# ecpoppenheimer/TensorFlowRayTrace

Hardware: AMD Instinct MI355X
Metric: ray-surface intersection tests/sec (fwd+bwd) (higher is better)
Workload: dtype f32 ray state, f32 filter + f64 decisions

## Files before the change

### tensorflowraytrace_amd/csrc/tfrt_trace3d.hip

```cpp
#include <vector>

#include <type_traits>
#include "tfrt_common.h"
#include "goal_finish.h"
#include "wave_schedule.h"

namespace tfrt {

constexpr int TILE = 512;
constexpr int KC = 24;

constexpr int ERR_CAPACITY = 1;


__global__ __launch_bounds__(BLOCK) void k_center(const double* __restrict__ fverts, int M,
                                                  double* __restrict__ c0, int32_t* nrays0, int n,
                                                  int32_t* tail8, unsigned int* scan_ticket) {
  if (nrays0 != nullptr) {
    if (threadIdx.x == 0) *nrays0 = n;
    if (threadIdx.x < 8) tail8[threadIdx.x] = 0;
    if (threadIdx.x == 0 && scan_ticket != nullptr) *scan_ticket = 0u;
  }
  __shared__ double red[WAVES][3];
  __shared__ double ctr[3];
// ... 1102 lines not shown
  group_walk<T, 1, false>(rays, stride, *n_ptr, last_tri, susphere, clsphere, csphere, crec, cface,
                          fverts, c0, prep, pstride, n_clusters, chunk_clusters, eps_int, eps_size,
                          eps_start, part_t, part_i, part_stride, catagory, rec_tri, rec_t, rec_cls,
                          blockcnt, nullptr, (int)blockIdx.x * BLOCK, -1);
}

template <typename T>
__global__ __launch_bounds__(BLOCK) void k_intersect_group_left(
    const T* __restrict__ rays, int64_t stride, const int32_t* __restrict__ n_ptr,
    const int32_t* __restrict__ last_tri, const float4* __restrict__ susphere,
    const float4* __restrict__ clsphere, const float4* __restrict__ csphere,
    const float4* __restrict__ crec, const int32_t* __restrict__ cface,
    const double* __restrict__ fverts, const double* __restrict__ c0, int n_clusters,
    int chunk_clusters, double eps_int, double eps_size, double eps_start,
    const int32_t* __restrict__ catagory, int32_t* __restrict__ rec_tri,
    double* __restrict__ rec_t, uint8_t* __restrict__ rec_cls,
    const int32_t* __restrict__ left_list, const int32_t* __restrict__ left_count,
    int32_t* __restrict__ hist) {
  const int n = *n_ptr;
  const int total = *left_count;
  for (int item = blockIdx.x; item * WAVES < total; item += gridDim.x) {
    const int k = item * WAVES + (int)(threadIdx.x >> 6);
    const int qwave = k < total ? left_list[k] : -1;
    group_walk<T, 1, true>(rays, stride, n, last_tri, susphere, clsphere, csphere, crec, cface,
                           fverts, c0, nullptr, 0, n_clusters, chunk_clusters, eps_int, eps_size,
                           eps_start, nullptr, nullptr, 0, catagory, rec_tri, rec_t, rec_cls,
                           nullptr, hist, 0, qwave);
    __syncthreads();
  }
}

constexpr int BEAM_SLIST = 64;
constexpr int BEAM_CLIST = 32;
constexpr int BEAM_FLIST = 192;
constexpr int BEAM_WIDE = 48;

struct Beam {
  float ox, oy, oz, wx, wy, wz, R0, S, tmin;
  float e1x, e1y, e1z, e2x, e2y, e2z;
  float R0b, tb;
  __device__ __forceinline__ float radius(float t, float pad) const {
    return fminf(R0 + S * (fabsf(t) + pad), R0b + S * (fabsf(t - tb) + pad));
  }
};

__device__ __forceinline__ bool beam_touch(const Beam& b, const float4 sp) {
  const float r = __builtin_amdgcn_sqrtf(sp.w) * 1.000002f;
  const float vx = sp.x - b.ox, vy = sp.y - b.oy, vz = sp.z - b.oz;
  const float t = vx * b.wx + vy * b.wy + vz * b.wz;
  const float v2 = vx * vx + vy * vy + vz * vz;
  const float B = r + b.radius(t, r);
  return (v2 - t * t <= B * B + 2e-6f * v2) && !(t + r < b.tmin);
}

__device__ __forceinline__ bool face_frame(const Beam& b, const float4 r0, const float4 r1,
                                           const float4 r2, const float es, float4 rec[4]) {
  const float n1 = fabsf(r1.x) + fabsf(r1.y) + fabsf(r1.z);
  const float n2 = fabsf(r2.x) + fabsf(r2.y) + fabsf(r2.z);
  const float scale = fabsf(r0.x) + fabsf(r0.y) + fabsf(r0.z) + fabsf(b.ox) + fabsf(b.oy) +
                      fabsf(b.oz) + n1 + n2;
  const float slack = 5.05f * es * (n1 + n2) + 8e-6f * scale;
  const float ax = r0.x - b.ox, ay = r0.y - b.oy, az = r0.z - b.oz;
  const float t0 = ax * b.wx + ay * b.wy + az * b.wz;
  const float t1 = t0 + (r1.x * b.wx + r1.y * b.wy + r1.z * b.wz);
  const float t2 = t0 + (r2.x * b.wx + r2.y * b.wy + r2.z * b.wz);
  const float tlo = fminf(t0, fminf(t1, t2)) - slack, thi = fmaxf(t0, fmaxf(t1, t2)) + slack;
  const float q0x = ax * b.e1x + ay * b.e1y + az * b.e1z, q0y = ax * b.e2x + ay * b.e2y + az * b.e2z;
  const float g1x = r1.x * b.e1x + r1.y * b.e1y + r1.z * b.e1z,
              g1y = r1.x * b.e2x + r1.y * b.e2y + r1.z * b.e2z;
  const float g2x = r2.x * b.e1x + r2.y * b.e1y + r2.z * b.e1z,
              g2y = r2.x * b.e2x + r2.y * b.e2y + r2.z * b.e2z;
  const float area = g1x * g2y - g1y * g2x;
  const float l1 = g1x * g1x + g1y * g1y, l2 = g2x * g2x + g2y * g2y;
  const bool flat = !(area * area > 1e-8f * l1 * l2);
  const float sg = area > 0.f ? 1.f : -1.f;
  auto edge = [&](float px, float py, float dx, float dy, float* nx, float* ny, float* c) {
    const float k = sg * __builtin_amdgcn_rsqf(dx * dx + dy * dy);
    *nx = dy * k;
    *ny = -dx * k;
    *c = -(*nx * px + *ny * py);
  };
  float nx0, ny0, c0, nx1, ny1, c1, nx2, ny2, c2;
  edge(q0x, q0y, g1x, g1y, &nx0, &ny0, &c0);
  edge(q0x + g1x, q0y + g1y, g2x - g1x, g2y - g1y, &nx1, &ny1, &c1);
  edge(q0x + g2x, q0y + g2y, -g2x, -g2y, &nx2, &ny2, &c2);
  if (flat) {
    nx0 = ny0 = nx1 = ny1 = nx2 = ny2 = 0.f;
    c0 = c1 = c2 = -INFINITY;
  }
  const float slack2 = 1.5f * slack;
  rec[0] = make_float4(nx0, ny0, c0, tlo);
  rec[1] = make_float4(nx1, ny1, c1, thi);
  rec[2] = make_float4(nx2, ny2, c2, 0.5f * (tlo + thi));
  rec[3] = make_float4(0.5001f * (thi - tlo), slack2, r0.w, 0.f);
  const float rho = (fminf(b.R0 + b.S * fmaxf(fabsf(tlo), fabsf(thi)),
                           b.R0b + b.S * fmaxf(fabsf(tlo - b.tb), fabsf(thi - b.tb))) +
                     slack2) * 1.0001f;
  return !(c0 > rho) && !(c1 > rho) && !(c2 > rho) && !(thi < b.tmin);
}

template <typename Op>
__device__ __forceinline__ float wave_reduce_f(float v, Op op) {
  auto dpp = [](float x, auto ctrl, auto row_mask) {
    return __int_as_float(__builtin_amdgcn_update_dpp(__float_as_int(x), __float_as_int(x),
                                                      decltype(ctrl)::value,
                                                      decltype(row_mask)::value, 0xF, false));
  };
  using std::integral_constant;
  v = op(v, dpp(v, integral_constant<int, 0xB1>{}, integral_constant<int, 0xF>{}));
  v = op(v, dpp(v, integral_constant<int, 0x4E>{}, integral_constant<int, 0xF>{}));
  v = op(v, dpp(v, integral_constant<int, 0x141>{}, integral_constant<int, 0xF>{}));
  v = op(v, dpp(v, integral_constant<int, 0x140>{}, integral_constant<int, 0xF>{}));
  v = op(v, dpp(v, integral_constant<int, 0x142>{}, integral_constant<int, 0xA>{}));
  v = op(v, dpp(v, integral_constant<int, 0x143>{}, integral_constant<int, 0xC>{}));
  return __int_as_float(__builtin_amdgcn_readlane(__float_as_int(v), 63));
}
__device__ __forceinline__ float wave_sum_f(float v) {
  return wave_reduce_f(v, [](float a, float b) { return a + b; });
}
__device__ __forceinline__ float wave_max_f(float v) {
  return wave_reduce_f(v, [](float a, float b) { return fmaxf(a, b); });
}
__device__ __forceinline__ float wave_min_f(float v) {
  return wave_reduce_f(v, [](float a, float b) { return fminf(a, b); });
}
#define TFRT_DPP_STEP4(OPA, OPB, OPC, OPD, CTRL)      \
  OPA " %0, %0, %0 " CTRL "\n\t" OPB " %1, %1, %1 " CTRL "\n\t" \
  OPC " %2, %2, %2 " CTRL "\n\t" OPD " %3, %3, %3 " CTRL "\n\t"
#define TFRT_DPP_ALL4(OPA, OPB, OPC, OPD)                                        \
  "s_nop 1\n\t"                                                                  \
  TFRT_DPP_STEP4(OPA, OPB, OPC, OPD, "quad_perm:[1,0,3,2] row_mask:0xf bank_mask:0xf") \
  TFRT_DPP_STEP4(OPA, OPB, OPC, OPD, "quad_perm:[2,3,0,1] row_mask:0xf bank_mask:0xf") \
  TFRT_DPP_STEP4(OPA, OPB, OPC, OPD, "row_half_mirror row_mask:0xf bank_mask:0xf")     \
  TFRT_DPP_STEP4(OPA, OPB, OPC, OPD, "row_mirror row_mask:0xf bank_mask:0xf")          \
  TFRT_DPP_STEP4(OPA, OPB, OPC, OPD, "row_bcast:15 row_mask:0xa bank_mask:0xf")        \
  TFRT_DPP_STEP4(OPA, OPB, OPC, OPD, "row_bcast:31 row_mask:0xc bank_mask:0xf")
__device__ __forceinline__ void wave_sum4(float& a, float& b, float& c, float& d) {
  __asm__ volatile(TFRT_DPP_ALL4("v_add_f32_dpp", "v_add_f32_dpp", "v_add_f32_dpp", "v_add_f32_dpp")
                   : "+v"(a), "+v"(b), "+v"(c), "+v"(d));
  a = __int_as_float(__builtin_amdgcn_readlane(__float_as_int(a), 63));
  b = __int_as_float(__builtin_amdgcn_readlane(__float_as_int(b), 63));
  c = __int_as_float(__builtin_amdgcn_readlane(__float_as_int(c), 63));
  d = __int_as_float(__builtin_amdgcn_readlane(__float_as_int(d), 63));
}
__device__ __forceinline__ void wave_max3_min(float& a, float& b, float& c, float& d) {
  __asm__ volatile(TFRT_DPP_ALL4("v_max_f32_dpp", "v_max_f32_dpp", "v_max_f32_dpp", "v_min_f32_dpp")
                   : "+v"(a), "+v"(b), "+v"(c), "+v"(d));
  a = __int_as_float(__builtin_amdgcn_readlane(__float_as_int(a), 63));
  b = __int_as_float(__builtin_amdgcn_readlane(__float_as_int(b), 63));
  c = __int_as_float(__builtin_amdgcn_readlane(__float_as_int(c), 63));
  d = __int_as_float(__builtin_amdgcn_readlane(__float_as_int(d), 63));
}

__device__ __forceinline__ float uniform_f(float v) {
  return __int_as_float(__builtin_amdgcn_readfirstlane(__float_as_int(v)));
}
__device__ __forceinline__ float bcast_f(float v, int src_lane) {
  return __int_as_float(__builtin_amdgcn_readlane(__float_as_int(v), src_lane));
}

template <typename U>
using LdsPtr = __attribute__((address_space(3))) U*;

template <typename RT>
__device__ __forceinline__ void beam_decide(const int nb, const int lane, LdsPtr<const uint32_t> x_pair,
                                         LdsPtr<const RT> rt, LdsPtr<unsigned long long> best_k,
                                         LdsPtr<int32_t> best_i, const double* __restrict__ fverts,
                                         const double eps_int, const double eps_size,
                                         const double eps_start) {
  bool have = false;
  unsigned long long key = 0, old = 0;
  int j = -1;
  const uint32_t xp = lane < nb ? x_pair[lane] : 0u;
  const int slot = (int)(xp & 63u);
  if (lane < nb) {
    double s[3], e[3];
#pragma unroll
    for (int k = 0; k < 3; ++k) {
      s[k] = static_cast<double>(rt[k * 64 + slot]);
      e[k] = static_cast<double>(rt[(3 + k) * 64 + slot]);
    }
    j = (int)(xp >> 6);
    old = best_k[slot];
    double P[9];
    const double* fp = fverts + 9 * (int64_t)j;
#pragma unroll
    for (int k = 0; k < 9; ++k) P[k] = fp[k];
    const TriHit h = exact_triangle(s, e, P, eps_int, eps_size, eps_start);
    if (h.valid) {
      have = true;
      key = dkey(h.ray_u);
    }
  }
  wave_fence();
  if (have) atomicMin((unsigned long long*)&best_k[slot], key);
  wave_fence();
  bool win = false;
  if (have) {
    const unsigned long long now = best_k[slot];
    win = key == now;
    if (win && now < old) best_i[slot] = 0x7FFFFFFF;
  }
  wave_fence();
  if (win) atomicMin((int32_t*)&best_i[slot], j);
  wave_fence();
}

template <typename RT>
struct BeamLds {
  uint16_t slist[BEAM_SLIST];
  uint16_t clist[BEAM_CLIST];
  uint32_t flist[BEAM_FLIST];
  uint32_t x_pair[192];
  float4 ftab[64][4];
  RT rtab[6][64];
  unsigned long long best_k[64];
  int32_t best_i[64];
};

struct BeamScene {
  const float4* susphere;
  const float4* clsphere;
  const float4* csphere;
  const float4* crec;
  const double* fverts;
  const double* c0;
  int n_clusters, n_super;
  double eps_int, eps_size, eps_start;
};

#ifdef TFRT_TICKS
#define TFRT_WI_ARG _wi
#else
#define TFRT_WI_ARG nullptr
#endif

template <typename T, typename RT>
__device__ __forceinline__ bool beam_pass(BeamLds<RT>& W, const BeamScene& g, const int lane,
                                          const int bundle, const bool live, const int skip,
                                          const bool first_pass, const int coherent_only,
                                          unsigned* _wi, unsigned* work = nullptr) {
  TFRT_TICK_INIT;
  const float4* __restrict__ susphere = g.susphere;
  const float4* __restrict__ clsphere = g.clsphere;
  const float4* __restrict__ csphere = g.csphere;
  const float4* __restrict__ crec = g.crec;
  const double* __restrict__ fverts = g.fverts;
  const double* __restrict__ c0 = g.c0;
  const int n_clusters = g.n_clusters, n_super = g.n_super;
  const double eps_int = g.eps_int, eps_size = g.eps_size, eps_start = g.eps_start;
  const float4 never = make_float4(0.f, 0.f, 0.f, -1.f);
  W.best_k[lane] = dkey(INFINITY);
  W.best_i[lane] = -1;
  const double cx = c0[0], cy = c0[1], cz = c0[2];
  const float cxf = uniform_f((float)cx), cyf = uniform_f((float)cy), czf = uniform_f((float)cz);
  auto rel = [](const RT v, const double c, const float cf) -> float {
    if constexpr (sizeof(T) <= 4) return (float)v - cf;
    else return (float)((double)v - c);
  };
  const float es_f = (float)eps_size;
  int xn = 0;

  auto decide = [&](const int nb) {
    TFRT_STAT(28, 1);
    TFRT_WAVE_NOTE(1, 1);
    wave_fence();
    beam_decide<RT>(nb, lane, (LdsPtr<const uint32_t>)&W.x_pair[0],
                    (LdsPtr<const RT>)&W.rtab[0][0], (LdsPtr<unsigned long long>)&W.best_k[0],
                    (LdsPtr<int32_t>)&W.best_i[0], fverts, eps_int, eps_size, eps_start);
  };

  TFRT_STAT(8, 1);
  constexpr int BEAM_ATTEMPTS = 20;
  TFRT_TICK(0);
  float gap = -1.f;
  unsigned long long cuts = 0ull;
  int lo = 0, attempts = 0;
  bool spread = false;
  while (lo < bundle) {
    ++attempts;
    TFRT_STAT(30, 1);
    TFRT_WAVE_NOTE(0, 1);
    const unsigned long long above = lo < 63 ? (cuts >> (lo + 1)) << (lo + 1) : 0ull;
    const int hi = above != 0ull ? __ffsll((long long)above) - 1 : bundle;
    const int len = hi - lo;
    wave_fence();
    RT own[6];
#pragma unroll
    for (int k = 0; k < 6; ++k) own[k] = W.rtab[k][lane];
    const float sx = rel(own[0], cx, cxf), sy = rel(own[1], cy, cyf), sz = rel(own[2], cz, czf);
    const float dx = (float)(own[3] - own[0]), dy = (float)(own[4] - own[1]),
                dz = (float)(own[5] - own[2]);
    const float len2 = dx * dx + dy * dy + dz * dz;
    const bool ok = live && len2 > 0.f && len2 < 3.0e38f;
    const float inv = ok ? __builtin_amdgcn_rsqf(len2) : 0.f;
    const float ux = dx * inv, uy = dy * inv, uz = dz * inv;
    const float rabs = fabsf(sx) + fabsf(sy) + fabsf(sz);
    const bool sel = ok && lane >= lo && lane < hi;
    const float4 su_first = lane < n_super ? susphere[lane] : never;
    const float cnt = (float)__popcll(__ballot(sel));
    bool narrow = true, brute = false;
    int ns = 0, nc = 0, nf = 0;
    Beam bm = {0.f, 0.f, 0.f, 0.f, 0.f, 1.f, 0.f, 0.f, -INFINITY, 1.f, 0.f, 0.f, 0.f, 1.f, 0.f,
               INFINITY, 0.f};
    float ray_t = 0.f, ray_dt = 0.f, ray_terr = 0.f;
    float Ax = 0.f, Ay = 0.f, Mx = 0.f, My = 0.f, Mlen = 0.f, Perr = 0.f, Pm = 0.f;
    if (cnt > 0.f) {
      float swx = sel ? ux : 0.f, swy = sel ? uy : 0.f, swz = sel ? uz : 0.f;
      float sox = sel ? sx : 0.f, soy = sel ? sy : 0.f, soz = sel ? sz : 0.f;
      float pad0 = 0.f, pad1 = 0.f;
      wave_sum4(swx, swy, swz, sox);
      wave_sum4(soy, soz, pad0, pad1);
      const float wl2 = swx * swx + swy * swy + swz * swz;
      narrow = wl2 > 0.49f * cnt * cnt;
      spread = !narrow;
      const float wi = narrow ? __builtin_amdgcn_rsqf(wl2) : 0.f;
      bm.wx = swx * wi; bm.wy = swy * wi; bm.wz = swz * wi;
      const float icnt = __builtin_amdgcn_rcpf(cnt);
      bm.ox = sox * icnt; bm.oy = soy * icnt; bm.oz = soz * icnt;
      const float cosk = ux * bm.wx + uy * bm.wy + uz * bm.wz;
      if (__any(sel && !(cosk > 0.7f))) narrow = false, spread = true;
      const float px = sx - bm.ox, py = sy - bm.oy, pz = sz - bm.oz;
      const float ts = px * bm.wx + py * bm.wy + pz * bm.wz;
      ray_t = ts;
      ray_dt = dx * bm.wx + dy * bm.wy + dz * bm.wz;
      ray_terr = 1e-5f * (rabs + fabsf(bm.ox) + fabsf(bm.oy) + fabsf(bm.oz));
      {
        const float f0 = fabsf(bm.wx), f1 = fabsf(bm.wy), f2 = fabsf(bm.wz);
        const bool k0 = f0 <= f1 && f0 <= f2, k1 = !k0 && f1 <= f2;
        const float kx = k0 ? 1.f : 0.f, ky = k1 ? 1.f : 0.f, kz = (!k0 && !k1) ? 1.f : 0.f;
        const float cxx = bm.wy * kz - bm.wz * ky, cyy = bm.wz * kx - bm.wx * kz,
                    czz = bm.wx * ky - bm.wy * kx;
        const float il = __builtin_amdgcn_rsqf(cxx * cxx + cyy * cyy + czz * czz);
        bm.e1x = cxx * il; bm.e1y = cyy * il; bm.e1z = czz * il;
        bm.e2x = bm.wy * bm.e1z - bm.wz * bm.e1y;
        bm.e2y = bm.wz * bm.e1x - bm.wx * bm.e1z;
        bm.e2z = bm.wx * bm.e1y - bm.wy * bm.e1x;
      }
      {
        const float idt = __builtin_amdgcn_rcpf(sel ? ray_dt : 1.f);
        Mx = (dx * bm.e1x + dy * bm.e1y + dz * bm.e1z) * idt;
        My = (dx * bm.e2x + dy * bm.e2y + dz * bm.e2z) * idt;
        const float p1 = px * bm.e1x + py * bm.e1y + pz * bm.e1z,
                    p2 = px * bm.e2x + py * bm.e2y + pz * bm.e2z;
        Ax = p1 - ts * Mx;
        Ay = p2 - ts * My;
        Mlen = __builtin_amdgcn_sqrtf(Mx * Mx + My * My) * 1.0001f;
        Pm = 2e-5f * (fabsf(Mx) + fabsf(My));
        Perr = 2e-5f * (fabsf(p1) + fabsf(p2) + fabsf(ts) * (fabsf(Mx) + fabsf(My)) + rabs +
                        fabsf(bm.ox) + fabsf(bm.oy) + fabsf(bm.oz));
      }
      float R0 = sel ? __builtin_amdgcn_sqrtf(Ax * Ax + Ay * Ay) : 0.f, S = sel ? Mlen : 0.f;
      float Lw = sel ? rabs : 0.f, tmin = sel ? ts : INFINITY;
      wave_max3_min(R0, S, Lw, tmin);
      Lw += fabsf(bm.ox) + fabsf(bm.oy) + fabsf(bm.oz);
      const float tb = -(bm.ox * bm.wx + bm.oy * bm.wy + bm.oz * bm.wz);
      float R0b = 0.f;
      if (sel) {
        const float bx = Ax + Mx * tb, by = Ay + My * tb;
        R0b = __builtin_amdgcn_sqrtf(bx * bx + by * by);
      }
      R0b = wave_max_f(R0b);
      bm.R0 = R0 * 1.001f + 4e-6f * Lw;
      bm.S = S * 1.001f + 2e-6f;
      bm.tb = tb;
      bm.R0b = R0b * 1.001f + 4e-6f * (Lw + fabsf(tb)) + 2e-6f * fabsf(tb) * S;
      if (!(bm.R0b < 3.0e38f)) bm.R0b = INFINITY;
      bm.tmin = (!first_pass && eps_start >= 0.0) ? tmin - 1e-5f * Lw - 1e-5f * fabsf(tmin)
                                                  : -INFINITY;
      if (!(bm.R0 < 3.0e38f && bm.S < 3.0e38f)) narrow = false;
      bm.ox = uniform_f(bm.ox); bm.oy = uniform_f(bm.oy); bm.oz = uniform_f(bm.oz);
      bm.wx = uniform_f(bm.wx); bm.wy = uniform_f(bm.wy); bm.wz = uniform_f(bm.wz);
      bm.R0 = uniform_f(bm.R0); bm.S = uniform_f(bm.S); bm.tmin = uniform_f(bm.tmin);
      bm.R0b = uniform_f(bm.R0b); bm.tb = uniform_f(bm.tb);
      bm.e1x = uniform_f(bm.e1x); bm.e1y = uniform_f(bm.e1y); bm.e1z = uniform_f(bm.e1z);
      bm.e2x = uniform_f(bm.e2x); bm.e2y = uniform_f(bm.e2y); bm.e2z = uniform_f(bm.e2z);
      TFRT_TICK(1);

      if (narrow) {
        float4 nxt = su_first;
        for (int b = 0; b < n_super; b += 64) {
          const int node = b + lane;
          const float4 cur = nxt;
          nxt = node + 64 < n_super ? susphere[node + 64] : never;
          const bool hit = beam_touch(bm, cur);
          const unsigned long long m = __ballot(hit);
          if (hit) {
            const int pos = ns + rank_below(m);
            if (pos < BEAM_SLIST) W.slist[pos] = (uint16_t)node;
          }
          ns += __popcll(m);
        }
        narrow = ns <= BEAM_SLIST && n_super <= 65536;
      }
      wave_fence();
      TFRT_TICK(2);
      if (narrow && ns > 0) {
        for (int b = 0; b < ns * SUPER; b += 64) {
          const int k = b + lane;
          bool hit = false;
          int cl = 0;
          if (k < ns * SUPER) {
            cl = (int)W.slist[k >> 3] * SUPER + (k & 7);
            if (cl < n_clusters) hit = beam_touch(bm, clsphere[cl]);
          }
          const unsigned long long m = __ballot(hit);
          if (hit) {
            const int pos = nc + rank_below(m);
            if (pos < BEAM_CLIST) W.clist[pos] = (uint16_t)cl;
          }
          nc += __popcll(m);
        }
        narrow = nc <= BEAM_CLIST && n_clusters <= 65536;
      }
      wave_fence();
      TFRT_TICK(3);
      if (narrow && nc > 0) {
        for (int b = 0; b < nc * CLUSTER; b += 64) {
          const int k = b + lane;
          bool hit = false;
          unsigned slot = 0;
          if (k < nc * CLUSTER) {
            slot = (unsigned)W.clist[k >> 4] * CLUSTER + (unsigned)(k & 15);
            hit = beam_touch(bm, csphere[slot]);
          }
          const unsigned long long m = __ballot(hit);
          if (hit) {
            const int pos = nf + rank_below(m);
            if (pos < BEAM_FLIST) W.flist[pos] = slot;
          }
          nf += __popcll(m);
        }
        narrow = nf <= BEAM_FLIST && !(nf > BEAM_WIDE && len > 8 && attempts <= 6);
      }
      wave_fence();
      TFRT_TICK(4);
    }
    if (!narrow) {
      TFRT_TICK(10);
      const bool hopeless = !coherent_only &&
                            ((len == bundle && (spread || (nc > 64 && nc > n_clusters / 4))) ||
                             attempts >= BEAM_ATTEMPTS);
      if (len > 1 && !hopeless) {
        if (cuts == 0ull) {
          const float su = sx * ux + sy * uy + sz * uz;
          const float fx = sx - su * ux, fy = sy - su * uy, fz = sz - su * uz;
          const float gx = fx - __shfl_up(fx, 1, 64), gy = fy - __shfl_up(fy, 1, 64),
                      gz = fz - __shfl_up(fz, 1, 64);
          const float hx = ux - __shfl_up(ux, 1, 64), hy = uy - __shfl_up(uy, 1, 64),
                      hz = uz - __shfl_up(uz, 1, 64);
          const bool prev_ok = __shfl_up(ok ? 1 : 0, 1, 64) != 0;
          gap = 0.f;
          if (ok && prev_ok && lane > 0)
            gap = gx * gx + gy * gy + gz * gz +
                  (sx * sx + sy * sy + sz * sz) * (hx * hx + hy * hy + hz * hz);
          if (!(gap >= 0.f)) gap = 0.f;
        }
        const bool inside = lane > lo && lane < hi;
        const float widest = wave_max_f(inside ? gap : -1.f);
        const unsigned long long at = __ballot(inside && gap == widest);
        const int g = (widest > 0.f && at != 0ull) ? __ffsll((long long)at) - 1 : lo + (len >> 1);
        cuts |= 1ull << g;
        continue;
      }
      if (len == 1 && !hopeless) {
        brute = true;
      } else {
        TFRT_STAT(ns > BEAM_SLIST ? 10 : (nc > BEAM_CLIST ? 11 : (nf > BEAM_FLIST ? 12 : 9)), 1);
        TFRT_STAT(15, lo);
        return false;
      }
    }

    TFRT_STAT(13, nf);
    TFRT_WAVE_NOTE(3, nf);
    TFRT_TICK(5);
    auto reach_now = [&]() {
      const double best = dkey_inv(W.best_k[lane]);
      const float bu = nextafterf((float)best, INFINITY) * ray_dt;
      return ray_t + bu + 1e-5f * fabsf(bu) + ray_terr;
    };
    float myreach = reach_now();
    bool queued = false;
    const int n_cand = brute ? n_clusters * CLUSTER : nf;
    int f0 = 0;
    do {
      const int nb = min(64, n_cand - f0);
      if (work != nullptr) work[1] += (unsigned)nb;
      float4 rec[4] = {never, never, never, never};
      bool touch = false;
      float tnear = INFINITY;
      bool cand = lane < nb;
      if (brute && cand) {
        const float4 sp = csphere[f0 + lane];
        const float vx = sp.x - bm.ox, vy = sp.y - bm.oy, vz = sp.z - bm.oz;
        const float vu = vx * bm.wx + vy * bm.wy + vz * bm.wz;
        const float v2 = vx * vx + vy * vy + vz * vz;
        const float rr = __builtin_amdgcn_sqrtf(sp.w) * 1.000002f + bm.radius(vu, 0.f);
        cand = v2 - vu * vu <= rr * rr + 4e-6f * v2;
      }
      if (cand) {
        const int64_t memb = brute ? (int64_t)(f0 + lane) : (int64_t)W.flist[f0 + lane];
        const float4 r0 = crec[3 * memb], r1 = crec[3 * memb + 1], r2 = crec[3 * memb + 2];
        touch = face_frame(bm, r0, r1, r2, es_f, rec) && __float_as_int(r0.w) >= 0;
        tnear = rec[0].w;
        if (tnear != tnear) tnear = -INFINITY;
        rec[0].w = tnear;
      }
      f0 += 64;
      const bool closing = f0 >= n_cand && hi == bundle;
      const unsigned long long tm = __ballot(touch);
      const int nt = __popcll(tm);
      int place = 0;
      for (unsigned long long rest = tm; rest != 0ull; rest &= rest - 1ull) {
        const int o = __ffsll((long long)rest) - 1;
        const float to = bcast_f(tnear, o);
        place += (to < tnear || (to == tnear && o < lane)) ? 1 : 0;
      }
      wave_fence();
      if (touch) {
        W.ftab[place][0] = rec[0];
        W.ftab[place][1] = rec[1];
        W.ftab[place][2] = rec[2];
        W.ftab[place][3] = rec[3];
      }
      wave_fence();
      TFRT_STAT(27, nt);
      TFRT_TICK(6);
      float span = -INFINITY;
      auto on_face = [&](const float word, const int b, int* j, float* thi) {
        const float tn = bcast_f(word, b + 3), tc = bcast_f(word, b + 11);
        *thi = bcast_f(word, b + 7);
        *j = __float_as_int(bcast_f(word, b + 14));
        const float ix = Ax + Mx * tc, iy = Ay + My * tc;
        const float room = Mlen * bcast_f(word, b + 12) + bcast_f(word, b + 13) + Perr + Pm * fabsf(tc);
        return sel && *j != skip && !(myreach < tn) &&
               !(bm.tmin > -INFINITY && *thi < ray_t - ray_terr) &&
               !(bcast_f(word, b) * ix + bcast_f(word, b + 1) * iy + bcast_f(word, b + 2) > room) &&
               !(bcast_f(word, b + 4) * ix + bcast_f(word, b + 5) * iy + bcast_f(word, b + 6) > room) &&
               !(bcast_f(word, b + 8) * ix + bcast_f(word, b + 9) * iy + bcast_f(word, b + 10) > room);
      };
      for (int c = 0;; c += 2) {
        const bool end = c >= nt;
        const bool two = c + 1 < nt;
        const float word =
            reinterpret_cast<const float*>(&W.ftab[end ? 0 : c][0])[lane & (two ? 31 : 15)];
        const float tn = end ? INFINITY : bcast_f(word, 3);
        const bool flush =
            end ? closing
                : (tn > span && __ballot(sel && !(queued || myreach < INFINITY)) == 0ull);
        while (xn >= 64 || (flush && xn > 0)) {
          const int nd = min(xn, 64);
          wave_fence();
          decide(nd);
          uint32_t tp = 0u, tq = 0u;
          if (lane < xn - nd) tp = W.x_pair[nd + lane];
          if (lane + 64 < xn - nd) tq = W.x_pair[nd + 64 + lane];
          wave_fence();
          if (lane < xn - nd) W.x_pair[lane] = tp;
          if (lane + 64 < xn - nd) W.x_pair[64 + lane] = tq;
          xn -= nd;
          wave_fence();
          if (xn == 0) queued = false;
          myreach = reach_now();
          TFRT_TICK(8);
        }
        if (end) break;
        if (__ballot(sel && !(myreach < tn)) == 0ull) {
          c = nt - 2;
          continue;
        }
        TFRT_STAT(29, two ? 2 : 1);
        TFRT_WAVE_NOTE(2, two ? 2 : 1);
        int ja, jb = -1;
        float thia, thib = -INFINITY;
        const bool keepa = on_face(word, 0, &ja, &thia);
        bool keepb = false;
        if (two) keepb = on_face(word, 16, &jb, &thib);
        span = fmaxf(span, fmaxf(thia, thib));
        const unsigned long long kma = __ballot(keepa), kmb = __ballot(keepb);
        const int na = __popcll(kma);
        if (keepa) W.x_pair[xn + rank_below(kma)] = ((uint32_t)ja << 6) | (uint32_t)lane;
        if (keepb) W.x_pair[xn + na + rank_below(kmb)] = ((uint32_t)jb << 6) | (uint32_t)lane;
        queued = queued || keepa || keepb;
        xn += na + __popcll(kmb);
        if (work != nullptr) work[0] += (unsigned)(na + __popcll(kmb));
        TFRT_STAT(14, na + __popcll(kmb));
        TFRT_TICK(7);
      }
    } while (f0 < n_cand);
    lo = hi;
  }
  wave_fence();
  return true;
}

template <typename T, int BW>
__global__ __launch_bounds__(64 * BW) void k_intersect_beam(
    const T* __restrict__ rays, int64_t stride, const int32_t* __restrict__ n_ptr,
    const int32_t* __restrict__ last_tri, BeamScene g, const int32_t* __restrict__ catagory,
    int32_t* __restrict__ rec_tri, double* __restrict__ rec_t, uint8_t* __restrict__ rec_cls,
    int32_t* __restrict__ hist, int32_t* __restrict__ left_list, int32_t* __restrict__ left_count,
    int32_t* __restrict__ left_total, int coherent_only, int bundle) {
  const int tid = threadIdx.x, lane = tid & 63, wave = tid >> 6;
  const int qwave = blockIdx.x * BW + wave;
  const int q = qwave * bundle + lane;
  const int n = *n_ptr;
  if (qwave * bundle >= n) return;
  TFRT_WAVE_BEGIN;

  using RT = std::conditional_t<sizeof(T) <= 4, float, double>;
  const int i = (lane < bundle && q < n) ? q : -1;
  const bool live = i >= 0;
  const int64_t ii = live ? i : 0;
  __shared__ BeamLds<RT> lds[BW];
  BeamLds<RT>& W = lds[wave];
#pragma unroll
  for (int k = 0; k < 6; ++k) W.rtab[k][lane] = static_cast<RT>(rays[k * stride + ii]);
  const int skip = (live && last_tri != nullptr) ? last_tri[ii] : -1;
  if (!beam_pass<T, RT>(W, g, lane, bundle, live, skip, last_tri == nullptr, coherent_only,
                        TFRT_WI_ARG)) {
    if (lane == 0) {
      left_list[atomicAdd(left_count, 1)] = qwave;
      atomicAdd(left_total, 1);
    }
    return;
  }
  wave_fence();

  int cls = -1;
  if (live) {
    const int bi = W.best_i[lane];
    cls = (bi < 0) ? CLS_DEAD : cat_to_cls(catagory[bi]);
    rec_tri[i] = bi;
    rec_t[i] = dkey_inv(W.best_k[lane]);
    rec_cls[i] = (uint8_t)cls;
  }
#pragma unroll
  for (int c = 0; c < 4; ++c) {
    const int cnt_c = __popcll(__ballot(cls == c));
    if (lane == c && cnt_c > 0) atomicAdd(&hist[((qwave * bundle) >> 8) * 4 + c], cnt_c);
  }
  TFRT_WAVE_END(qwave);
}


__global__ __launch_bounds__(BLOCK) void k_classify3d(
    const int32_t* __restrict__ n_ptr, int chunks, const double* __restrict__ part_t,
    const int32_t* __restrict__ part_i, int64_t part_stride,
    const int32_t* __restrict__ catagory, int32_t* __restrict__ rec_tri,
    double* __restrict__ rec_t, uint8_t* __restrict__ rec_cls, int32_t* __restrict__ blockcnt) {
  const int n = *n_ptr;
  const int base = blockIdx.x * BLOCK;
  if (base >= n) return;
  const int i = base + threadIdx.x;
  int cls = -1;
  if (i < n) {
    double bt = INFINITY;
    int bi = -1;
    for (int c = 0; c < chunks; ++c) {
      const double t = part_t[c * part_stride + i];
      const int pi = part_i[c * part_stride + i];
      if (t < bt || (t == bt && pi >= 0 && pi < bi)) {
        bt = t;
        bi = pi;
      }
    }
    cls = (bi < 0) ? CLS_DEAD : cat_to_cls(catagory[bi]);
    rec_tri[i] = bi;
    rec_t[i] = bt;
    rec_cls[i] = (uint8_t)cls;
  }
  __shared__ int wc[WAVES][4];
  const int wave = threadIdx.x >> 6;
#pragma unroll
  for (int c = 0; c < 4; ++c) {
    const unsigned long long m = __ballot(cls == c);
    if (lane_id() == 0) wc[wave][c] = __popcll(m);
  }
  __syncthreads();
  if (threadIdx.x < 4) {
    int s = 0;
    for (int w = 0; w < WAVES; ++w) s += wc[w][threadIdx.x];
    blockcnt[blockIdx.x * 4 + threadIdx.x] = s;
  }
}


__global__ __launch_bounds__(1024) void k_scan3d_one(const int32_t* __restrict__ n_ptr,
                                                 const int32_t* __restrict__ blockcnt,
                                                 int32_t* __restrict__ blockoff,
                                                 int32_t* __restrict__ pass_counts,
                                                 int32_t* __restrict__ totals,
                                                 int32_t* __restrict__ n_next,
                                                 unsigned long long* __restrict__ n_tests,
                                                 int M) {
  const int n = *n_ptr;
  const int nblk = (n + BLOCK - 1) / BLOCK;
  __shared__ int total[4];
  scan_rows_one<4>(blockcnt, blockoff, nblk, total);
  if (threadIdx.x < 4) {
    const int c = threadIdx.x;
    pass_counts[c] = total[c];
    pass_counts[4 + c] = totals[c];
    totals[c] += total[c];
  }
  if (threadIdx.x == 0) {
    *n_next = total[CLS_ACTIVE];
    *n_tests += (unsigned long long)n * (unsigned long long)M;
  }
}

constexpr int SCAN_GRID_MIN_ROWS = 8192;
__global__ __launch_bounds__(1024) void k_scan3d(const int32_t* __restrict__ n_ptr,
                                                 const int32_t* __restrict__ blockcnt,
                                                 int32_t* __restrict__ blockoff,
                                                 int32_t* __restrict__ rowtot,
                                                 int32_t* __restrict__ rowbase,
                                                 unsigned int* __restrict__ ticket,
                                                 int32_t* __restrict__ pass_counts,
                                                 int32_t* __restrict__ totals,
                                                 int32_t* __restrict__ n_next,
                                                 unsigned long long* __restrict__ n_tests,
                                                 int M) {
  const int n = *n_ptr;
  const int nblk = (n + BLOCK - 1) / BLOCK;
  __shared__ int total[4];
  if (!scan_rows_grid<4>(blockcnt, blockoff, nblk, rowtot, rowbase, ticket, total)) return;
  if (threadIdx.x < 4) {
    const int c = threadIdx.x;
    pass_counts[c] = total[c];
// ... 2583 lines not shown
```

### tensorflowraytrace_amd/csrc/trace_math.h

```cpp
#pragma once
#include <math.h>

#if defined(__HIPCC__)
#define TFRT_HD __host__ __device__ __forceinline__
#else
#define TFRT_HD inline
#endif

namespace tfrt {

constexpr int CLS_ACTIVE = 0;
constexpr int CLS_FINISHED = 1;
constexpr int CLS_STOPPED = 2;
constexpr int CLS_DEAD = 3;

constexpr int CAT_OPTICAL = 0, CAT_STOP = 1, CAT_TARGET = 2;

struct TriHit {
  double ray_u, trig_u, trig_v;
  bool valid;
};

TFRT_HD TriHit exact_triangle(const double s[3], const double e[3], const double P[9],
                              double eps_int, double eps_size, double eps_start) {
#pragma clang fp contract(off)
  const double a = s[0] - e[0], d = s[1] - e[1], h = s[2] - e[2];
  const double b = P[3] - P[0], f = P[4] - P[1], k = P[5] - P[2];
  const double c = P[6] - P[0], g = P[7] - P[1], l = P[8] - P[2];
  const double q = s[0] - P[0], r = s[1] - P[1], t = s[2] - P[2];

  const double den = a * g * k + b * d * l + c * f * h - a * f * l - b * g * h - c * d * k;
  const double nr = b * l * r + c * f * t + g * k * q - b * g * t - c * k * r - f * l * q;
  const double nu = a * g * t + c * h * r + d * l * q - a * l * r - c * d * t - g * h * q;
  const double nv = a * k * r + b * d * t + f * h * q - a * f * t - b * h * r - d * k * q;

  TriHit o;
  bool valid = fabs(den) >= eps_int;
  const double sd = valid ? den : 1.0;
  o.ray_u = nr / sd;
  o.trig_u = nu / sd;
  o.trig_v = nv / sd;
  valid = valid && (o.trig_u >= -eps_size);
  valid = valid && (o.trig_v >= -eps_size);
  valid = valid && (o.trig_u + o.trig_v <= 1.0 + eps_size);
  valid = valid && (o.ray_u >= eps_start);
  o.valid = valid;
  return o;
}

TFRT_HD void hit_point(const double s[3], const double e[3], double ray_u, double h[3]) {
#pragma clang fp contract(off)
  h[0] = s[0] - ray_u * (s[0] - e[0]);
  h[1] = s[1] - ray_u * (s[1] - e[1]);
  h[2] = s[2] - ray_u * (s[2] - e[2]);
}

TFRT_HD double advance(double origin, double L, double dir) {
#pragma clang fp contract(off)
  return origin + L * dir;
}

TFRT_HD double advance_between(double s, double L, double e) {
#pragma clang fp contract(off)
  return s + L * (e - s);
}

TFRT_HD void cross3(const double a[3], const double b[3], double o[3]) {
#pragma clang fp contract(off)
  o[0] = a[1] * b[2] - a[2] * b[1];
  o[1] = a[2] * b[0] - a[0] * b[2];
  o[2] = a[0] * b[1] - a[1] * b[0];
}

TFRT_HD double dot3(const double a[3], const double b[3]) {
#pragma clang fp contract(off)
  return a[0] * b[0] + a[1] * b[1] + a[2] * b[2];
}

TFRT_HD void face_normal(const double P[9], double N[3], double C[3], double* clen) {
#pragma clang fp contract(off)
  const double A[3] = {P[3] - P[0], P[4] - P[1], P[5] - P[2]};
  const double B[3] = {P[6] - P[3], P[7] - P[4], P[8] - P[5]};
  cross3(A, B, C);
  const double len = sqrt(dot3(C, C));
  *clen = len;
  N[0] = C[0] / len;
  N[1] = C[1] / len;
  N[2] = C[2] / len;
}

TFRT_HD double l2_normalize3(const double v[3], double o[3]) {
#pragma clang fp contract(off)
  double sq = dot3(v, v);
  if (sq < 1e-12) sq = 1e-12;
  const double inv = 1.0 / sqrt(sq);
  o[0] = v[0] * inv;
  o[1] = v[1] * inv;
  o[2] = v[2] * inv;
  return inv;
}

struct Snell3 {
  double u[3], n[3];
  double nu, eta, k;
  bool reflect;
  double w[3];
};

TFRT_HD void snell_normal(const double P[9], double n[3]) {
  double N[3], C[3], clen;
  face_normal(P, N, C, &clen);
  l2_normalize3(N, n);
}

TFRT_HD void snell_ratios(double n_in, double n_out, double* n1, double* n2) {
#pragma clang fp contract(off)
  const bool in_safe = n_in != 0.0, out_safe = n_out != 0.0;
  const double nis = in_safe ? n_in : 1.0, nos = out_safe ? n_out : 1.0;
  *n1 = out_safe ? nis / nos : 0.0;
  *n2 = in_safe ? nos / nis : 0.0;
}

TFRT_HD Snell3 snell3d_core(const double s[3], const double h[3], const double un[3], double n1,
                            double n2, bool mirror) {
#pragma clang fp contract(off)
  Snell3 o;
  const double r[3] = {h[0] - s[0], h[1] - s[1], h[2] - s[2]};
  l2_normalize3(r, o.u);
  o.n[0] = un[0];
  o.n[1] = un[1];
  o.n[2] = un[2];
  o.nu = dot3(o.n, o.u);
  const bool internal = o.nu > 0.0;
  o.eta = internal ? n1 : n2;
  const double nu_eta = o.eta * o.nu;
  o.k = 1.0 - o.eta * o.eta + nu_eta * nu_eta;
  const bool tir = o.k < 0.0;
  o.reflect = tir || mirror;
  if (o.reflect) {
    for (int i = 0; i < 3; ++i) o.w[i] = -2.0 * o.nu * o.n[i] + o.u[i];
  } else {
    const double sg = (o.nu > 0.0) ? 1.0 : ((o.nu < 0.0) ? -1.0 : 0.0);
    const double alpha = sg * sqrt(o.k) - nu_eta;
    for (int i = 0; i < 3; ++i) o.w[i] = alpha * o.n[i] + o.eta * o.u[i];
  }
  return o;
}

TFRT_HD Snell3 snell3d_unit(const double s[3], const double h[3], const double un[3],
                            double n_in, double n_out) {
  double n1, n2;
  snell_ratios(n_in, n_out, &n1, &n2);
  return snell3d_core(s, h, un, n1, n2, n_in == 0.0);
}

TFRT_HD Snell3 snell3d(const double s[3], const double h[3], const double norm[3],
                       double n_in, double n_out) {
  double un[3];
  l2_normalize3(norm, un);
  return snell3d_unit(s, h, un, n_in, n_out);
}

TFRT_HD double fmod_floor(double x, double m) {
  double r = fmod(x, m);
  if (r != 0.0 && ((r < 0.0) != (m < 0.0))) r += m;
  return r;
}

TFRT_HD double snell2d_angle(double xs, double ys, double xe, double ye, double norm,
                             double n_in, double n_out) {
#pragma clang fp contract(off)
  const double PI = 3.141592653589793;
  norm = fmod_floor(norm, 2 * PI);
  double ray_angle = atan2(ys - ye, xs - xe);
  ray_angle = fmod_floor(ray_angle, 2 * PI);
  double theta1 = norm - ray_angle;
  if (theta1 > PI) theta1 = theta1 - 2 * PI;
  if (theta1 < -PI) theta1 = theta1 + 2 * PI;
  const bool internal = fabs(theta1) >= PI / 2;
  const bool in_safe = n_in != 0.0, out_safe = n_out != 0.0;
  const double nis = in_safe ? n_in : 1.0, nos = out_safe ? n_out : 1.0;
  const double n1 = out_safe ? nis / nos : 0.0;
  const double n2 = in_safe ? nos / nis : 0.0;
  const double n = internal ? n1 : n2;
  if (!internal) norm = norm + PI;
  if (internal) theta1 = theta1 + PI;
  const double theta2 = n * sin(theta1);
  if (fabs(theta2) <= 1.0 && n != 0.0) return norm - asin(theta2);
  return norm + theta1 + PI;
}

TFRT_HD double adj_rcp(double x) {
#if defined(__HIP_DEVICE_COMPILE__)
  double r = __builtin_amdgcn_rcp(x);
  r = __builtin_fma(__builtin_fma(-x, r, 1.0), r, r);
  r = __builtin_fma(__builtin_fma(-x, r, 1.0), r, r);
  return r;
#else
  return 1.0 / x;
#endif
// ... 179 lines not shown
```

Before: 131800 billion.

## Rewrite face culling with DPP row broadcasts and merge wave reductions

Replaces the per-face culling math, which used many readlane broadcasts, with an inline-asm sequence built on row_newbcast DPP. Each 16-lane row can then evaluate its own face record, so the second face comes from a separate 16-float load. The 64-wide ftab gets one extra padding row so that load stays in bounds. Wave reductions are regrouped so the padded sum4 and the separate R0b max collapse into a sum2+max and a single max3_min. nextafterf is replaced by a bit-trick next_up_f. The gain is fewer scalar readlanes and DPP passes in the inner candidate loop, at the cost of hand-written asm with hazard nops and stricter register-lifetime assumptions.

```diff
diff --git a/tensorflowraytrace_amd/csrc/tfrt_trace3d.hip b/tensorflowraytrace_amd/csrc/tfrt_trace3d.hip
--- a/tensorflowraytrace_amd/csrc/tfrt_trace3d.hip
+++ b/tensorflowraytrace_amd/csrc/tfrt_trace3d.hip
@@ -1278,6 +1278,53 @@
   d = __int_as_float(__builtin_amdgcn_readlane(__float_as_int(d), 63));
 }
 
+#define TFRT_DPP_STEP3(OPA, OPB, OPC, CTRL) \
+  OPA " %0, %0, %0 " CTRL "\n\t" OPB " %1, %1, %1 " CTRL "\n\t" OPC " %2, %2, %2 " CTRL "\n\t"
+#define TFRT_DPP_ALL3(OPA, OPB, OPC)                                        \
+  "s_nop 1\n\t"                                                             \
+  TFRT_DPP_STEP3(OPA, OPB, OPC, "quad_perm:[1,0,3,2] row_mask:0xf bank_mask:0xf") \
+  TFRT_DPP_STEP3(OPA, OPB, OPC, "quad_perm:[2,3,0,1] row_mask:0xf bank_mask:0xf") \
+  TFRT_DPP_STEP3(OPA, OPB, OPC, "row_half_mirror row_mask:0xf bank_mask:0xf")     \
+  TFRT_DPP_STEP3(OPA, OPB, OPC, "row_mirror row_mask:0xf bank_mask:0xf")          \
+  TFRT_DPP_STEP3(OPA, OPB, OPC, "row_bcast:15 row_mask:0xa bank_mask:0xf")        \
+  TFRT_DPP_STEP3(OPA, OPB, OPC, "row_bcast:31 row_mask:0xc bank_mask:0xf")
+__device__ __forceinline__ void wave_sum2_max(float& a, float& b, float& c) {
+  __asm__ volatile(TFRT_DPP_ALL3("v_add_f32_dpp", "v_add_f32_dpp", "v_max_f32_dpp")
+                   : "+v"(a), "+v"(b), "+v"(c));
+  a = __int_as_float(__builtin_amdgcn_readlane(__float_as_int(a), 63));
+  b = __int_as_float(__builtin_amdgcn_readlane(__float_as_int(b), 63));
+  c = __int_as_float(__builtin_amdgcn_readlane(__float_as_int(c), 63));
+}
+
+#define TFRT_BCAST(K) " row_newbcast:" #K " row_mask:0xf bank_mask:0xf\n\t"
+__device__ __forceinline__ void face_edges(const float word, const float Ax, const float Ay,
+                                           const float Mx, const float My, const float Mlen,
+                                           const float Perr, const float Pm, float& room,
+                                           float& e0, float& e1, float& e2) {
+  float ix, iy;
+  __asm__ volatile(
+      "s_nop 1\n\t"
+      "v_mov_b32_dpp %3, %6" TFRT_BCAST(11)
+      "v_mov_b32_dpp %0, %6" TFRT_BCAST(13)
+      "v_fma_f32 %5, %3, %10, %8\n\t"
+      "v_fma_f32 %4, %3, %9, %7\n\t"
+      "v_fmac_f32_dpp %0, %6, %11" TFRT_BCAST(12)
+      "v_mul_f32_dpp %1, %6, %5" TFRT_BCAST(1)
+      "v_mul_f32_dpp %2, %6, %5" TFRT_BCAST(5)
+      "v_add_f32 %0, %12, %0\n\t"
+      "v_fma_f32 %0, %13, |%3|, %0\n\t"
+      "v_fmac_f32_dpp %1, %6, %4" TFRT_BCAST(0)
+      "v_fmac_f32_dpp %2, %6, %4" TFRT_BCAST(4)
+      "v_mul_f32_dpp %3, %6, %5" TFRT_BCAST(9)
+      "v_add_f32_dpp %1, %6, %1" TFRT_BCAST(2)
+      "v_add_f32_dpp %2, %6, %2" TFRT_BCAST(6)
+      "v_fmac_f32_dpp %3, %6, %4" TFRT_BCAST(8)
+      "s_nop 1\n\t"
+      "v_add_f32_dpp %3, %6, %3" TFRT_BCAST(10)
+      : "=&v"(room), "=&v"(e0), "=&v"(e1), "=&v"(e2), "=&v"(ix), "=&v"(iy)
+      : "v"(word), "v"(Ax), "v"(Ay), "v"(Mx), "v"(My), "v"(Mlen), "v"(Perr), "v"(Pm));
+}
+
 __device__ __forceinline__ float uniform_f(float v) {
   return __int_as_float(__builtin_amdgcn_readfirstlane(__float_as_int(v)));
 }
@@ -1338,7 +1385,7 @@
   uint16_t clist[BEAM_CLIST];
   uint32_t flist[BEAM_FLIST];
   uint32_t x_pair[192];
-  float4 ftab[64][4];
+  float4 ftab[65][4];
   RT rtab[6][64];
   unsigned long long best_k[64];
   int32_t best_i[64];
@@ -1434,9 +1481,9 @@
     if (cnt > 0.f) {
       float swx = sel ? ux : 0.f, swy = sel ? uy : 0.f, swz = sel ? uz : 0.f;
       float sox = sel ? sx : 0.f, soy = sel ? sy : 0.f, soz = sel ? sz : 0.f;
-      float pad0 = 0.f, pad1 = 0.f;
+      float Lw = sel ? rabs : 0.f;
       wave_sum4(swx, swy, swz, sox);
-      wave_sum4(soy, soz, pad0, pad1);
+      wave_sum2_max(soy, soz, Lw);
       const float wl2 = swx * swx + swy * swy + swz * swz;
       narrow = wl2 > 0.49f * cnt * cnt;
       spread = !narrow;
@@ -1477,8 +1524,7 @@
                         fabsf(bm.ox) + fabsf(bm.oy) + fabsf(bm.oz));
       }
       float R0 = sel ? __builtin_amdgcn_sqrtf(Ax * Ax + Ay * Ay) : 0.f, S = sel ? Mlen : 0.f;
-      float Lw = sel ? rabs : 0.f, tmin = sel ? ts : INFINITY;
-      wave_max3_min(R0, S, Lw, tmin);
+      float tmin = sel ? ts : INFINITY;
       Lw += fabsf(bm.ox) + fabsf(bm.oy) + fabsf(bm.oz);
       const float tb = -(bm.ox * bm.wx + bm.oy * bm.wy + bm.oz * bm.wz);
       float R0b = 0.f;
@@ -1486,7 +1532,7 @@
         const float bx = Ax + Mx * tb, by = Ay + My * tb;
         R0b = __builtin_amdgcn_sqrtf(bx * bx + by * by);
       }
-      R0b = wave_max_f(R0b);
+      wave_max3_min(R0, S, R0b, tmin);
       bm.R0 = R0 * 1.001f + 4e-6f * Lw;
       bm.S = S * 1.001f + 2e-6f;
       bm.tb = tb;
@@ -1603,7 +1649,7 @@
     TFRT_TICK(5);
     auto reach_now = [&]() {
       const double best = dkey_inv(W.best_k[lane]);
-      const float bu = nextafterf((float)best, INFINITY) * ray_dt;
+      const float bu = next_up_f((float)best) * ray_dt;
       return ray_t + bu + 1e-5f * fabsf(bu) + ray_terr;
     };
     float myreach = reach_now();
@@ -1654,23 +1700,21 @@
       TFRT_STAT(27, nt);
       TFRT_TICK(6);
       float span = -INFINITY;
-      auto on_face = [&](const float word, const int b, int* j, float* thi) {
-        const float tn = bcast_f(word, b + 3), tc = bcast_f(word, b + 11);
-        *thi = bcast_f(word, b + 7);
-        *j = __float_as_int(bcast_f(word, b + 14));
-        const float ix = Ax + Mx * tc, iy = Ay + My * tc;
-        const float room = Mlen * bcast_f(word, b + 12) + bcast_f(word, b + 13) + Perr + Pm * fabsf(tc);
-        return sel && *j != skip && !(myreach < tn) &&
-               !(bm.tmin > -INFINITY && *thi < ray_t - ray_terr) &&
-               !(bcast_f(word, b) * ix + bcast_f(word, b + 1) * iy + bcast_f(word, b + 2) > room) &&
-               !(bcast_f(word, b + 4) * ix + bcast_f(word, b + 5) * iy + bcast_f(word, b + 6) > room) &&
-               !(bcast_f(word, b + 8) * ix + bcast_f(word, b + 9) * iy + bcast_f(word, b + 10) > room);
+      auto on_face = [&](const float word, int* j, float* thi) {
+        const float tn = bcast_f(word, 3);
+        *thi = bcast_f(word, 7);
+        *j = __float_as_int(bcast_f(word, 14));
+        float room, e0, e1, e2;
+        face_edges(word, Ax, Ay, Mx, My, Mlen, Perr, Pm, room, e0, e1, e2);
+        const bool behind = bm.tmin > -INFINITY && *thi < ray_t - ray_terr;
+        return (sel & (*j != skip) & !(myreach < tn) & !behind) &
+               (!(e0 > room) & !(e1 > room) & !(e2 > room));
       };
       for (int c = 0;; c += 2) {
         const bool end = c >= nt;
         const bool two = c + 1 < nt;
-        const float word =
-            reinterpret_cast<const float*>(&W.ftab[end ? 0 : c][0])[lane & (two ? 31 : 15)];
+        const float* recs = reinterpret_cast<const float*>(&W.ftab[end ? 0 : c][0]) + (lane & 15);
+        const float word = recs[0], word2 = recs[16];
         const float tn = end ? INFINITY : bcast_f(word, 3);
         const bool flush =
             end ? closing
@@ -1700,9 +1744,9 @@
         TFRT_WAVE_NOTE(2, two ? 2 : 1);
         int ja, jb = -1;
         float thia, thib = -INFINITY;
-        const bool keepa = on_face(word, 0, &ja, &thia);
+        const bool keepa = on_face(word, &ja, &thia);
         bool keepb = false;
-        if (two) keepb = on_face(word, 16, &jb, &thib);
+        if (two) keepb = on_face(word2, &jb, &thib);
         span = fmaxf(span, fmaxf(thia, thib));
         const unsigned long long kma = __ballot(keepa), kmb = __ballot(keepb);
         const int na = __popcll(kma);
diff --git a/tensorflowraytrace_amd/csrc/trace_math.h b/tensorflowraytrace_amd/csrc/trace_math.h
--- a/tensorflowraytrace_amd/csrc/trace_math.h
+++ b/tensorflowraytrace_amd/csrc/trace_math.h
@@ -46,6 +46,16 @@
   valid = valid && (o.ray_u >= eps_start);
   o.valid = valid;
   return o;
+}
+
+TFRT_HD float next_up_f(float x) {
+  x += 0.0f;
+  unsigned b;
+  __builtin_memcpy(&b, &x, 4);
+  const unsigned up = b + (unsigned)(((int)b >> 31) | 1);
+  float y;
+  __builtin_memcpy(&y, &up, 4);
+  return x < INFINITY ? y : x;
 }
 
 TFRT_HD void hit_point(const double s[3], const double e[3], double ray_u, double h[3]) {
```

Result: faster. 138200 billion, median of 6 (+4.9%).
